# kaleo996/F5E-TTS

Measured on AMD Instinct MI355X. Metric: mel_frames_per_sec, higher is better.
Workload: dtype bf16; 1 GPU; C2: F5TTS_v1_Base random-init, batch 1 per GPU, N_ref=188 N=469 frames, euler NFE=32, CFG=2.0 (cond+uncond batched), sway=-1.0, hipGraph ODE loop, HIP log-mel front-end + Vocos decode on GPU; parallelism=replica x1 (utterance sharding, no collective on the data path)

## Files before the change

f5e-tts_amd/csrc/attention.hip:

```cpp
#include <cstdlib>
#include "attention_step.h"

namespace {

struct AttnArgs {
  const bf16* q; const bf16* k; const bf16* v;
  bf16* o; int ldo;
  const int* kv_len;
  int S, H, rows_per_seq, n_pad;
  int n_main;
  F5ePrefetch pf;
};

template <int NSPLIT>
__global__ __launch_bounds__(NSPLIT * 64, 2) void attn_fwd_kernel(AttnArgs a) {
  __shared__ __attribute__((aligned(16))) float red[(NSPLIT > 1 ? NSPLIT - 1 : 1) * 64 * 34];

  const int lane = threadIdx.x & 63;
  const int wave = __builtin_amdgcn_readfirstlane(threadIdx.x >> 6);
  const int ql = lane & 31, hh = lane >> 5;
  if ((int)blockIdx.x >= a.n_main) {
    f5e_prefetch_run<NSPLIT * 64>(a.pf, (int)blockIdx.x - a.n_main, threadIdx.x, red);
    return;
  }

  const int qtiles = (a.rows_per_seq + 31) / 32;
  int bid = blockIdx.x;
  {
    const int nblk = a.n_main;
    const int q8 = nblk >> 3, r8 = nblk & 7;
    const int xcd = bid & 7, idx = bid >> 3;
    bid = (xcd < r8 ? xcd * (q8 + 1) : r8 * (q8 + 1) + (xcd - r8) * q8) + idx;
  }
  const int qt = bid % qtiles;
  bid /= qtiles;
  const int head = bid % a.H;
  const int seq = bid / a.H;
  const size_t sh = (size_t)seq * a.H + head;
  const int kv_len = a.kv_len ? min(a.kv_len[seq], a.rows_per_seq) : a.rows_per_seq;
  const int ntiles = (kv_len + 63) / 64;

  const bf16* Qg = a.q + sh * a.n_pad * 64;
  const bf16* Kg = a.k + sh * a.n_pad * 64;
  const bf16* Vg = a.v + sh * a.n_pad * 64;

  bf16x8 qf[4];
#pragma unroll
  for (int ks = 0; ks < 4; ++ks) qf[ks] = *(const bf16x8*)(Qg + ((size_t)(qt * 4 + ks) * 32 + ql) * 16 + hh * 8);

  bf16x8 kf[2][4], vf[2][2][2];
  auto load_tile = [&](int t64) {
#pragma unroll
    for (int t = 0; t < 2; ++t) {
      const size_t tile = (size_t)t64 * 2 + t;
#pragma unroll
      for (int ks = 0; ks < 4; ++ks) kf[t][ks] = *(const bf16x8*)(Kg + ((tile * 4 + ks) * 32 + ql) * 16 + hh * 8);
#pragma unroll
      for (int s = 0; s < 2; ++s)
#pragma unroll
        for (int dt = 0; dt < 2; ++dt)
          vf[t][s][dt] = *(const bf16x8*)(Vg + ((((tile * 2 + s) * 2 + dt) * 32 + ql) * 2 + hh) * 8);
    }
  };

  f32x16 oacc[2], minit;
  float m_run, l_val;
  bf16x8 ck[2][4], cv[2][2][2];
  int t64;
  auto advance = [&]() -> int {
#pragma unroll
    for (int t = 0; t < 2; ++t) {
#pragma unroll
      for (int ks = 0; ks < 4; ++ks) ck[t][ks] = kf[t][ks];
#pragma unroll
      for (int s = 0; s < 2; ++s)
#pragma unroll
        for (int dt = 0; dt < 2; ++dt) cv[t][s][dt] = vf[t][s][dt];
    }
    const int cur = t64;
    t64 += NSPLIT;
    if (t64 < ntiles) load_tile(t64);
    return cur;
  };
  auto pass_begin = [&]() {
#pragma unroll
    for (int r = 0; r < 16; ++r) { oacc[0][r] = 0.f; oacc[1][r] = 0.f; minit[r] = 0.f; }
    m_run = -INFINITY;
    l_val = 0.f;
    t64 = wave;
    if (t64 < ntiles) load_tile(t64);
  };
  auto checked_tile = [&](bool first) {
    const int cur = advance();
    f32x16 st[2];
    auto qk = [&](f32x16 (&d)[2], const f32x16& c) {
#pragma unroll
      for (int t = 0; t < 2; ++t) {
        d[t] = __builtin_amdgcn_mfma_f32_32x32x16_bf16(ck[t][0], qf[0], c, 0, 0, 0);
#pragma unroll
        for (int ks = 1; ks < 4; ++ks) d[t] = __builtin_amdgcn_mfma_f32_32x32x16_bf16(ck[t][ks], qf[ks], d[t], 0, 0, 0);
      }
    };
    softmax_step(qk, first, cur * 64 + 64 > kv_len, cur * 64 + 4 * hh, kv_len, st, minit, m_run, l_val, oacc);
#pragma unroll
    for (int t = 0; t < 2; ++t)
#pragma unroll
      for (int s = 0; s < 2; ++s) {
        bf16x8 pf;
#pragma unroll
        for (int j = 0; j < 8; ++j) pf[j] = (bf16)st[t][8 * s + j];
#pragma unroll
        for (int dt = 0; dt < 2; ++dt)
          oacc[dt] = __builtin_amdgcn_mfma_f32_32x32x16_bf16(cv[t][s][dt], pf, oacc[dt], 0, 0, 0);
      }
  };

  pass_begin();
  if (t64 < ntiles) checked_tile(true);
  const int nfull = (ntiles * 64 > kv_len) ? ntiles - 1 : ntiles;
  while (t64 < nfull) {
    advance();
    auto kfrag = [&](int t, int ks) { return ck[t][ks]; };
    auto vfrag = [&](int t, int s, int dt) { return cv[t][s][dt]; };
    fast_step(kfrag, vfrag, qf, minit, l_val, oacc);
  }
  if (t64 < ntiles) checked_tile(false);
  if (__builtin_amdgcn_ballot_w64(!accum_finite(l_val, oacc)) != 0) {
    pass_begin();
    bool first = true;
    while (t64 < ntiles) { checked_tile(first); first = false; }
  }

  float l_run = add_xor32(l_val);
  if (NSPLIT > 1) {
    if (wave > 0) {
      f32x4* dq = (f32x4*)(red + (wave - 1) * 64 * 34);
#pragma unroll
      for (int g = 0; g < 4; ++g) {
        dq[g * 64 + lane] = f32x4{oacc[0][4 * g], oacc[0][4 * g + 1], oacc[0][4 * g + 2], oacc[0][4 * g + 3]};
        dq[(4 + g) * 64 + lane] = f32x4{oacc[1][4 * g], oacc[1][4 * g + 1], oacc[1][4 * g + 2], oacc[1][4 * g + 3]};
      }
      *(f32x2*)(red + (wave - 1) * 64 * 34 + 64 * 32 + lane * 2) = f32x2{m_run, l_run};
    }
    __syncthreads();
    if (wave > 0) return;
#pragma unroll
    for (int w = 1; w < NSPLIT; ++w) {
      const f32x4* sq = (const f32x4*)(red + (w - 1) * 64 * 34);
      const f32x2 ml = *(const f32x2*)(red + (w - 1) * 64 * 34 + 64 * 32 + lane * 2);
      const float m_new = fmaxf(m_run, ml[0]);
      const float fa = fast_exp2(m_run - m_new), fb = fast_exp2(ml[0] - m_new);
#pragma unroll
      for (int g = 0; g < 4; ++g) {
        const f32x4 s0 = sq[g * 64 + lane], s1 = sq[(4 + g) * 64 + lane];
#pragma unroll
        for (int r = 0; r < 4; ++r) {
          oacc[0][4 * g + r] = oacc[0][4 * g + r] * fa + s0[r] * fb;
          oacc[1][4 * g + r] = oacc[1][4 * g + r] * fa + s1[r] * fb;
        }
      }
      l_run = l_run * fa + ml[1] * fb;
      m_run = m_new;
    }
  }

  {
    const float inv = l_run > 0.f ? 1.0f / l_run : 0.f;
    char* stg = (char*)red;
    if (NSPLIT > 1) asm volatile("s_waitcnt lgkmcnt(0)" ::: "memory");
#pragma unroll
    for (int dt = 0; dt < 2; ++dt)
#pragma unroll
      for (int g = 0; g < 4; ++g)
        *(bf16x4*)(stg + ql * 144 + 64 * dt + 16 * g + 8 * hh) =
            f2bf4(oacc[dt][4 * g] * inv, oacc[dt][4 * g + 1] * inv, oacc[dt][4 * g + 2] * inv, oacc[dt][4 * g + 3] * inv);
    asm volatile("s_waitcnt lgkmcnt(0)" ::: "memory");
#pragma unroll
    for (int it = 0; it < 4; ++it) {
      const int r = it * 8 + (lane >> 3), c = lane & 7;
      const int q_row = qt * 32 + r;
      const uint4 v = *(const uint4*)(stg + r * 144 + c * 16);
      if (q_row < a.rows_per_seq)
        *(uint4*)(a.o + ((size_t)seq * a.rows_per_seq + q_row) * a.ldo + head * 64 + c * 8) = v;
    }
  }
}


template <int NST, int OCC>
__global__ __launch_bounds__(256, OCC) void attn_fwd_lds_kernel(AttnArgs a) {
  constexpr int TILE_BYTES = 16384;
  extern __shared__ __attribute__((aligned(16))) char smem[];

  const int tid = threadIdx.x;
  const int lane = tid & 63;
  const int wave = __builtin_amdgcn_readfirstlane(tid >> 6);
  const int ql = lane & 31, hh = lane >> 5;

  const int qblocks = (a.rows_per_seq + 127) / 128;
  int bid = blockIdx.x;
  {
    const int nblk = gridDim.x;
    const int q8 = nblk >> 3, r8 = nblk & 7;
    const int xcd = bid & 7, idx = bid >> 3;
    bid = (xcd < r8 ? xcd * (q8 + 1) : r8 * (q8 + 1) + (xcd - r8) * q8) + idx;
  }
  const int qb = bid % qblocks;
  bid /= qblocks;
  const int head = bid % a.H;
  const int seq = bid / a.H;
  const size_t sh = (size_t)seq * a.H + head;
  const int kv_len = a.kv_len ? min(a.kv_len[seq], a.rows_per_seq) : a.rows_per_seq;
  const int ntiles = (kv_len + 63) / 64;

  const bf16* Qg = a.q + sh * a.n_pad * 64;
  const char* Kg = (const char*)(a.k + sh * a.n_pad * 64);
  const char* Vg = (const char*)(a.v + sh * a.n_pad * 64);

  const int qt = min(qb * 4 + wave, a.n_pad / 32 - 1);
  bf16x8 qf[4];
#pragma unroll
  for (int ks = 0; ks < 4; ++ks) qf[ks] = *(const bf16x8*)(Qg + ((size_t)(qt * 4 + ks) * 32 + ql) * 16 + hh * 8);

  const int src16 = ((lane & 31) * 2 + (lane >> 5)) * 16;
  auto stage = [&](int buf, int t64) {
    char* dst = smem + buf * TILE_BYTES;
#pragma unroll
    for (int j = 0; j < 2; ++j) {
      const int off = (wave * 64 + 256 * j) * 16;
      __builtin_amdgcn_global_load_lds((const __attribute__((address_space(1))) void*)(Kg + (size_t)t64 * 8192 + off + src16),
                                       (__attribute__((address_space(3))) void*)(dst + off), 16, 0, 0);
      __builtin_amdgcn_global_load_lds((const __attribute__((address_space(1))) void*)(Vg + (size_t)t64 * 8192 + off + src16),
                                       (__attribute__((address_space(3))) void*)(dst + 8192 + off), 16, 0, 0);
    }
  };

  f32x16 oacc[2], minit;
  float m_run, l_val;

  int buf = 0, nbuf = NST - 1;
  auto tile_wait = [&](int t64) -> const char* {
    const int young = min(NST - 2, ntiles - 1 - t64);
    if (young >= 2) asm volatile("s_waitcnt vmcnt(8) lgkmcnt(0)" ::: "memory");
    else if (young == 1) asm volatile("s_waitcnt vmcnt(4) lgkmcnt(0)" ::: "memory");
    else asm volatile("s_waitcnt vmcnt(0) lgkmcnt(0)" ::: "memory");
    __builtin_amdgcn_s_barrier();
    return smem + buf * TILE_BYTES;
  };
  auto tile_stage = [&](int t64) {
    if (t64 + NST - 1 < ntiles) stage(nbuf, t64 + NST - 1);
    buf = (buf == NST - 1) ? 0 : buf + 1;
    nbuf = (nbuf == NST - 1) ? 0 : nbuf + 1;
  };
  auto tile_begin = [&](int t64) -> const char* {
    const char* Ks = tile_wait(t64);
    tile_stage(t64);
    return Ks;
  };
  auto pass_begin = [&]() {
#pragma unroll
    for (int r = 0; r < 16; ++r) { oacc[0][r] = 0.f; oacc[1][r] = 0.f; minit[r] = 0.f; }
    m_run = -INFINITY;
    l_val = 0.f;
    buf = 0;
    nbuf = NST - 1;
#pragma unroll
    for (int t = 0; t < NST - 1; ++t)
      if (t < ntiles) stage(t, t);
  };
  auto checked_tile = [&](int t64) {
    const char* Ks = tile_begin(t64);
    const char* Vs = Ks + 8192;
    f32x16 st[2];
    auto qk = [&](f32x16 (&d)[2], const f32x16& c) {
#pragma unroll
      for (int ks = 0; ks < 4; ++ks)
#pragma unroll
        for (int t = 0; t < 2; ++t) {
          const bf16x8 kf = *(const bf16x8*)(Ks + (t * 4 + ks) * 1024 + lane * 16);
          d[t] = __builtin_amdgcn_mfma_f32_32x32x16_bf16(kf, qf[ks], ks == 0 ? c : d[t], 0, 0, 0);
        }
    };
    softmax_step(qk, t64 == 0, t64 * 64 + 64 > kv_len, t64 * 64 + 4 * hh, kv_len, st, minit, m_run, l_val, oacc);
#pragma unroll
    for (int t = 0; t < 2; ++t)
#pragma unroll
      for (int s = 0; s < 2; ++s) {
        bf16x8 pf;
#pragma unroll
        for (int j = 0; j < 8; ++j) pf[j] = (bf16)st[t][8 * s + j];
#pragma unroll
        for (int dt = 0; dt < 2; ++dt) {
          const bf16x8 vf = *(const bf16x8*)(Vs + (((t * 2 + s) * 2 + dt) * 1024) + lane * 16);
          oacc[dt] = __builtin_amdgcn_mfma_f32_32x32x16_bf16(vf, pf, oacc[dt], 0, 0, 0);
        }
      }
  };

  pass_begin();
  if (ntiles > 0) checked_tile(0);
  const int nfull = (ntiles > 0 && ntiles * 64 > kv_len) ? ntiles - 1 : ntiles;
  for (int t64 = 1; t64 < nfull; ++t64) {
    const char* Ks = tile_wait(t64);
    const char* Vs = Ks + 8192;
    bf16x8 kf0[4];
#pragma unroll
    for (int ks = 0; ks < 4; ++ks) kf0[ks] = *(const bf16x8*)(Ks + ks * 1024 + lane * 16);
    tile_stage(t64);
    auto kfrag = [&](int t, int ks) { return t == 0 ? kf0[ks] : *(const bf16x8*)(Ks + (t * 4 + ks) * 1024 + lane * 16); };
    auto vfrag = [&](int t, int s, int dt) { return *(const bf16x8*)(Vs + (((t * 2 + s) * 2 + dt) * 1024) + lane * 16); };
    fast_step(kfrag, vfrag, qf, minit, l_val, oacc);
  }
  if (nfull < ntiles && ntiles > 1) checked_tile(ntiles - 1);
  if (__syncthreads_or(!accum_finite(l_val, oacc))) {
    pass_begin();
    for (int t64 = 0; t64 < ntiles; ++t64) checked_tile(t64);
  }

  const float l_run = add_xor32(l_val);
  const int q_row = (qb * 4 + wave) * 32 + ql;
  if (q_row < a.rows_per_seq) {
    const float inv = l_run > 0.f ? 1.0f / l_run : 0.f;
    bf16* op = a.o + ((size_t)seq * a.rows_per_seq + q_row) * a.ldo + head * 64 + 4 * hh;
#pragma unroll
    for (int dt = 0; dt < 2; ++dt)
#pragma unroll
      for (int g = 0; g < 4; ++g) {
        *(bf16x4*)(op + dt * 32 + 8 * g) = f2bf4(oacc[dt][4 * g] * inv, oacc[dt][4 * g + 1] * inv,
                                                   oacc[dt][4 * g + 2] * inv, oacc[dt][4 * g + 3] * inv);
      }
  }
}

}

int f5e_flash_attn_pf(hipStream_t st, const void* q, const void* k, const void* v, void* o, int ldo, const int* kv_len,
                      int S, int H, int rows_per_seq, int n_pad, int splits, const F5ePrefetch* pf) {
  F5E_REQUIRE(q && k && v && o, "flash_attn: null pointer");
  F5E_REQUIRE(S > 0 && H > 0 && rows_per_seq > 0, "flash_attn: empty problem");
  F5E_REQUIRE(n_pad % 64 == 0 && n_pad >= rows_per_seq, "flash_attn: n_pad=%d must be a multiple of 64 and >= %d",
              n_pad, rows_per_seq);
  F5E_REQUIRE(ldo % 8 == 0 && ldo >= H * 64 && ((uintptr_t)o & 15) == 0, "flash_attn: bad ldo=%d / output alignment", ldo);
  AttnArgs a{};
  a.q = (const bf16*)q; a.k = (const bf16*)k; a.v = (const bf16*)v; a.o = (bf16*)o; a.ldo = ldo;
  a.kv_len = kv_len; a.S = S; a.H = H; a.rows_per_seq = rows_per_seq; a.n_pad = n_pad;
  const int grid = ((rows_per_seq + 31) / 32) * H * S;
  a.n_main = grid;
  if (splits == -1 || (splits == 0 && grid >= 8192)) {
    const int g128 = ((rows_per_seq + 127) / 128) * H * S;
#ifdef F5E_TOOLS
    static const int variant = getenv("F5E_ATTN_VARIANT") ? atoi(getenv("F5E_ATTN_VARIANT")) : 0;
    if (variant == 33) {
      static F5eDeviceOnce once33;
      hipLaunchKernelGGL((attn_fwd_lds_kernel<3, 3>), dim3(g128), dim3(256), 3 * 16384, st, a);
    } else if (variant == 23) {
      hipLaunchKernelGGL((attn_fwd_lds_kernel<2, 3>), dim3(g128), dim3(256), 2 * 16384, st, a);
    } else if (variant == 42) {
      hipLaunchKernelGGL((attn_fwd_lds_kernel<4, 2>), dim3(g128), dim3(256), 4 * 16384, st, a);
    } else
#endif
    hipLaunchKernelGGL((attn_fwd_lds_kernel<2, 4>), dim3(g128), dim3(256), 2 * 16384, st, a);
    F5E_LAUNCH_CHECK("flash_attn_lds");
    return F5E_OK;
  }
  if (splits <= 0) {
    const int ktiles = (rows_per_seq + 63) / 64;
    splits = grid > 2 * f5e_cu_count() ? 1 : 4;
    while (splits > 1 && splits > ktiles) splits >>= 1;
  }
  switch (splits) {
    case 1: {
      const int npf = f5e_prefetch_wgs(pf);
      if (npf) a.pf = *pf;
      hipLaunchKernelGGL(attn_fwd_kernel<1>, dim3(grid + npf), dim3(64), 0, st, a);
      break;
    }
    case 2: {
      const int npf = f5e_prefetch_wgs(pf);
      if (npf) a.pf = *pf;
      hipLaunchKernelGGL(attn_fwd_kernel<2>, dim3(grid + npf), dim3(128), 0, st, a);
      break;
    }
    case 4: {
      const int npf = f5e_prefetch_wgs(pf);
      if (npf) a.pf = *pf;
      hipLaunchKernelGGL(attn_fwd_kernel<4>, dim3(grid + npf), dim3(256), 0, st, a);
      break;
    }
    default: F5E_REQUIRE(false, "flash_attn: splits must be 0 (auto), -1 (LDS-shared), 1, 2 or 4");
  }
  F5E_LAUNCH_CHECK("flash_attn");
  return F5E_OK;
}

extern "C" int f5e_flash_attn(hipStream_t st, const void* q, const void* k, const void* v, void* o, int ldo,
                              const int* kv_len, int S, int H, int rows_per_seq, int n_pad, int splits) {
  return f5e_flash_attn_pf(st, q, k, v, o, ldo, kv_len, S, H, rows_per_seq, n_pad, splits, nullptr);
}
```

include/f5e_abi.h:

```cpp
#ifndef F5E_ABI_H_
#define F5E_ABI_H_

#ifdef __cplusplus
extern "C" {
#endif

#define F5E_ABI_VERSION 2

#if defined(__GNUC__)
#define F5E_API __attribute__((visibility("default")))
#else
#define F5E_API
#endif

enum { F5E_OK = 0, F5E_ERR_BAD_SHAPE = -1, F5E_ERR_UNSUPPORTED = -2, F5E_ERR_HIP = -3 };

enum { F5E_ACT_NONE = 0, F5E_ACT_SILU = 1, F5E_ACT_GELU_ERF = 2, F5E_ACT_GELU_TANH = 3, F5E_ACT_RELU = 4, F5E_ACT_MISH = 5 };

#ifdef F5E_STREAM_T
typedef F5E_STREAM_T f5e_stream;
#else
typedef void* f5e_stream;
#endif

F5E_API int f5e_abi_version(void);
F5E_API const char* f5e_last_error(void);
F5E_API int f5e_check_device(void);


F5E_API int f5e_gemm_bf16_bias(f5e_stream st, const void* A, int lda, const void* W, int ldw, const float* bias, void* out,
                       int ldo, int M, int N, int K, int act, int out_f32, int tile_hint);

F5E_API int f5e_gemm_bf16_gate_residual(f5e_stream st, const void* A, int lda, const void* W, int ldw, const float* bias,
                                float* resid, int ldr, const float* gate, int gate_stride, int gate_rows,
                                const int* eval_ptr, int eval_stride, int rows_per_seq, const int* seq_len, int M,
                                int N, int K, int tile_hint);

F5E_API int f5e_gemm_bf16_qkv_rope(f5e_stream st, const void* A, int lda, const void* W, int ldw, const float* bias, void* q,
                           void* k, void* vt, int n_pad, int heads, int rope_heads, const float* cos_sin,
                           const float* q_norm_w, const float* k_norm_w, int rows_per_seq, int M, int K,
                           int tile_hint);

typedef struct f5e_ln_fuse {
  const float* stats; int parts;
  const float* c; const float* d; int cd_stride; int cd_rows; int cd_eval_stride;
  const int* eval_ptr; int rows_per_seq; float eps;
  void* xs_out; int ld_xs; const float* next_scale;
  float* stats_out;
  float* row_mean;
} f5e_ln_fuse;

F5E_API int f5e_gemm_bf16_bias_ln(f5e_stream st, const void* A, int lda, const void* W, int ldw, const float* bias, void* out,
                          int ldo, int M, int N, int K, int act, int out_f32, int tile_hint, const f5e_ln_fuse* ln);
F5E_API int f5e_gemm_bf16_gate_residual_ln(f5e_stream st, const void* A, int lda, const void* W, int ldw, const float* bias,
                                   float* resid, int ldr, const float* gate, int gate_stride, int gate_rows,
                                   const int* eval_ptr, int eval_stride, int rows_per_seq, const int* seq_len, int M,
                                   int N, int K, int tile_hint, const f5e_ln_fuse* ln);
F5E_API int f5e_gemm_bf16_qkv_rope_ln(f5e_stream st, const void* A, int lda, const void* W, int ldw, const float* bias,
                              void* q, void* k, void* vt, int n_pad, int heads, int rope_heads, const float* cos_sin,
                              const float* q_norm_w, const float* k_norm_w, int rows_per_seq, int M, int K,
                              int tile_hint, const f5e_ln_fuse* ln);


F5E_API int f5e_flash_attn(f5e_stream st, const void* q, const void* k, const void* vt, void* o, int ldo, const int* kv_len,
                   int S, int H, int rows_per_seq, int n_pad, int splits);

F5E_API int f5e_joint_attn(f5e_stream st, const void* qx, const void* kx, const void* vx, const void* qc, const void* kc,
                   const void* vc, void* o_x, int ldo_x, void* o_c, int ldo_c, const int* kv_len, int S, int H, int N,
                   int n_pad_x, int Nt, int n_pad_c, int splits);


F5E_API int f5e_layernorm(f5e_stream st, const float* x, int ldx, void* y, int ldy, int y_bf16, const float* gamma,
                  const float* beta, const float* scale, const float* shift, int mod_stride, int mod_rows,
                  int rows_per_seq, const int* eval_ptr, int eval_stride, int rows, int D, float eps);

F5E_API int f5e_adaln_pre(f5e_stream st, const float* x, int ldx, void* xs, int ld_xs, const float* scale, int mod_stride,
                  int mod_rows, int rows_per_seq, const int* eval_ptr, int eval_stride, float* stats, int parts,
                  float* row_mean, int rows, int D);

F5E_API int f5e_l2norm(f5e_stream st, const float* x, int ldx, void* y, int ldy, int y_bf16, const float* g, int rows, int D);

F5E_API int f5e_grn(f5e_stream st, const float* x, float* y, float* gx_ws, const float* gamma, const float* beta, int B, int T,
            int C);


F5E_API int f5e_gemm_f32(f5e_stream st, const float* A, int lda, int a_rows, int a_act, const float* W, int ldw,
                 const float* bias, int act, const float* ch_scale, const float* addend, int ld_add, int add_rows,
                 const float* row_scale, float* out, int ldo, void* out_bf16, int ldo_bf16, int M, int N, int K);


F5E_API int f5e_convpos(f5e_stream st, const void* x, int ldx, const void* w_packed, const float* bias, int mode,
                void* out_bf16, int ldo, float* out_f32, int ldo32, const float* resid, int ldr, int S, int N, int D,
                int groups);

F5E_API int f5e_dwconv7(f5e_stream st, const float* x, const float* w_t, const float* bias, float* y, int B, int T, int C);

F5E_API int f5e_im2col(f5e_stream st, const float* x, float* col, int B, int T, int Cin, int ksize, int pad);


F5E_API int f5e_sinus_embed(f5e_stream st, const float* t, const float* freqs, float* out, int E, int dim, float scale);
F5E_API int f5e_rope_table(f5e_stream st, const float* inv_freq, float* out, int N, int half);
F5E_API int f5e_text_gather(f5e_stream st, const int* ids, const float* table, const float* pos, const float* keep, float* out,
                    int B, int N, int TD, int max_pos, int table_rows);
F5E_API int f5e_ode_update(f5e_stream st, const float* pred, long long branch_stride, int mode, float w0, float w1,
                   const float* base, float* dst, float* traj, const float* coef, int* eval_ptr, unsigned* done_ctr,
                   long long n);
F5E_API int f5e_ode_update_traj(f5e_stream st, const float* pred, long long branch_stride, int mode, float w0, float w1,
                        const float* base, float* dst, float* traj, long long traj_stride, int traj_div,
                        const float* coef, int* eval_ptr, unsigned* done_ctr, long long n);
F5E_API int f5e_advance_eval(f5e_stream st, int* eval_ptr);
F5E_API int f5e_stitch(f5e_stream st, const float* cond, const float* y, const unsigned char* mask, float* out, long long rows,
               int C);
F5E_API int f5e_cast_bf16(f5e_stream st, const float* x, void* y, long long n);
F5E_API int f5e_cast_f32(f5e_stream st, const void* x, float* y, long long n);
F5E_API int f5e_axpby(f5e_stream st, const float* x, const float* y, float* out, float a, float b, float c, long long n);
F5E_API int f5e_vq_eval(f5e_stream st, const float* logits, int ld, const float* vars, int combine_groups, float* out,
                int* targets, float* stats, int rows, int groups, int num_vars, int var_dim);

F5E_API int f5e_mas_workspace_bytes(int B, int Ty, int Tx, unsigned long long* bytes_out_host);
F5E_API int f5e_mas_path(f5e_stream st, const float* logp, long long batch_stride, int ld, const int* t_y, const int* t_x,
                 int* token_of_frame, int* durations, void* workspace, unsigned long long workspace_bytes, int B, int Ty,
                 int Tx);

F5E_API int f5e_resample(f5e_stream st, const float* x, long long ld_x, const float* bank, int orig, int new_, int width,
                 float* y, long long ld_y, int B, int n, int n_out);

F5E_API int f5e_ctc_align_workspace_bytes(int B, int T, int L, unsigned long long* bytes_out_host);
F5E_API int f5e_ctc_align(f5e_stream st, const float* scores, long long batch_stride, int ld, const int* labels, int ld_labels,
                  const int* t_len, const int* l_len, int blank, int* align, int* tok_start, int* tok_end, float* score,
                  void* workspace, unsigned long long workspace_bytes, int B, int T, int L, int V);

F5E_API int f5e_ctc_greedy(f5e_stream st, const float* scores, long long batch_stride, int ld, const int* t_len, int blank,
                   int pad_id, int* hyp, int* hyp_len, float* frame_logp, int B, int T, int V);

F5E_API int f5e_ctc_beam_workspace_bytes(int B, int T, int beam, unsigned long long* bytes_out_host);
F5E_API int f5e_ctc_beam(f5e_stream st, const float* scores, long long batch_stride, int ld, const int* t_len, int blank,
                 int beam, int* hyp, int ld_hyp, int* hyp_len, float* score, void* workspace,
                 unsigned long long workspace_bytes, int B, int T, int V);

F5E_API int f5e_ctc_beam_state_bytes(int B, int T_cap, int chunk_cap, int beam, unsigned long long* bytes_out_host);
F5E_API int f5e_ctc_beam_state_init(f5e_stream st, void* state, unsigned long long state_bytes, int B, int T_cap,
                            int chunk_cap, int beam);
F5E_API int f5e_ctc_beam_chunk(f5e_stream st, const float* scores, long long batch_stride, int ld, const int* n_frames,
                       int T_chunk, int V, int blank, int beam, void* state, unsigned long long state_bytes, int* hyp,
                       int ld_hyp, int* hyp_len, float* score, int B, int T_cap, int chunk_cap);

F5E_API int f5e_token_logp(f5e_stream st, const float* logits, long long ld, const int* target, float* out, long long rows,
                   int V);
F5E_API int f5e_log_softmax_rows(f5e_stream st, const float* x, long long ldx, float* out, long long ldo, long long rows,
                         int V);


F5E_API int f5e_stft_logmel(f5e_stream st, const float* wav, int nw, int ldw, const float* window, const float* twiddle,
                    const float* fb, float* out, int B, int n_fft, int hop, int n_mels);
F5E_API int f5e_stft_logmel_banded(f5e_stream st, const float* wav, int nw, int ldw, const float* window, const float* twiddle,
                           const float* fb_compact, const int* fb_band, int nnz, float* out, int B, int n_fft, int hop,
                           int n_mels);
F5E_API int f5e_stft_logmel_banded_ex(f5e_stream st, const float* wav, int nw, int ldw, const float* window,
                              const float* twiddle, const float* fb_compact, const int* fb_band, int nnz, float* out, int B,
                              int n_fft, int hop, int n_mels, int pad_left, int T, float mag_eps);
F5E_API int f5e_istft_head(f5e_stream st, const float* z, int ldz, const float* window, const float* twiddle, float* frames_ws,
                   float* out, int B, int T, int n_fft, int hop);


F5E_API int f5e_bigvgan_act(f5e_stream st, const float* x, void* y, int out_f32, const float* alpha, const float* inv_beta,
                    const float* f_up, const float* f_dn, int B, int L, int C);
F5E_API int f5e_bigvgan_conv(f5e_stream st, const void* x, const void* w_packed, const float* bias, const float* resid,
                     float* out, float* sum, float sum_scale, int sum_init, int B, int L, int Cin, int Cin_pad, int N,
                     int ksz, int dil, int pad);
F5E_API int f5e_bigvgan_post(f5e_stream st, const float* a, const float* w, const float* bias, float* out, int B, int L, int C,
                     int ksz, int use_tanh);


F5E_API int f5e_kaldi_fbank(f5e_stream st, const float* wav, int nw, int ldw, const float* window, const float* twiddle,
                    const float* fb, float* out, int B, int win, int shift, int n_mels, float in_scale, float preemph,
                    float eps);
F5E_API int f5e_glu(f5e_stream st, const float* x, int ldx, float* y, int ldy, long long rows, int C);
F5E_API int f5e_dwconv(f5e_stream st, const float* x, const float* w_t, const float* bias, const float* keep, float* y, int B,
               int T, int C, int K);
F5E_API int f5e_softmax_rows(f5e_stream st, const float* x, int ldx, float* y, int ldy, const int* kv_len, long long rows,
                     int rows_per_seq, int L, float scale);
F5E_API int f5e_dwconv_stream(f5e_stream st, const float* x, const float* w_t, const float* bias, const float* fill, float* y,
                      int B, int T, int C, int K, int causal, int chunk);
F5E_API int f5e_relpos_attn(f5e_stream st, const float* qu, int ldq, const float* k, int ldk, const float* pos, int ldp,
                    const float* v, int ldv, float* out, int ldo, const int* kv_len, int B, int T, int H, int dk,
                    int q_begin, int chunk, int left_chunks, float scale);
F5E_API int f5e_mha_f32(f5e_stream st, const float* q, int ldq, const float* k, int ldk, const float* v, int ldv, float* out,
                int ldo, const int* kv_len, int B, int Tq, int Tk, int H, int dk, int causal, float scale);

F5E_API int f5e_attn_decode_f32(f5e_stream st, const float* qkv, int ld_qkv, float* kc, float* vc, long long row_stride,
                        int pos_stride, const int* anc, int ld_anc, float* out, int ldo, int R, int Umax, int H, int dk, int p,
                        float scale);
F5E_API int f5e_beam_step(f5e_stream st, const float* logits, long long ld_logits, float* score, const int* hyp_in,
                  const int* anc_in, int* hyp_out, int* anc_out, int ld, int* last, int* alive, int* done_at, int B, int V,
                  int beam, int p, int eos);


typedef struct f5e_dit_block_weights {
  const void* w_qkv;  const float* b_qkv;
  const void* w_out;  const float* b_out;
  const void* w_ff1;  const float* b_ff1;
  const void* w_ff2;  const float* b_ff2;
  const float* q_norm_w; const float* k_norm_w;
} f5e_dit_block_weights;

typedef struct f5e_dit_plan {
  int S, B, N, n_pad, D, H, rope_heads, FF, L, mel;
  int mod_rows;
  const float* y;
  const float* w_x; int ldw_x;
  const float* in_const;
  const void* convpos_w1; const float* convpos_b1;
  const void* convpos_w2; const float* convpos_b2;
  int convpos_groups;
  const float* rope_cs;
  const int* seq_len;
  const float* mod;
  const int* eval_ptr;
  const f5e_dit_block_weights* blocks;
  const void* w_proj; const float* b_proj;
  const float* w_skip;
  float* skip_res; float* skip_tmp;
  float* h0; void* h0_bf16; void* c1;
  float* x;
  void* hn;
  void* q; void* k; void* vt;
  void* ao;
  void* ff;
  float* pred;
  void* timer;
  int timer_op;
  int fuse_ln;
  float* ln_stats;
  float* ln_rowmean;
  const float* cd;
  int cd_stride;
  int mall_prefetch;
} f5e_dit_plan;

enum { F5E_WS_H0 = 0, F5E_WS_H0_BF16, F5E_WS_C1, F5E_WS_X, F5E_WS_HN, F5E_WS_Q, F5E_WS_K, F5E_WS_VT, F5E_WS_AO, F5E_WS_FF,
       F5E_WS_PRED, F5E_WS_LN_STATS, F5E_WS_SKIP_RES, F5E_WS_SKIP_TMP, F5E_WS_LN_ROWMEAN, F5E_WS_COUNT };
typedef struct f5e_dit_workspace {
  int n_pad;
  unsigned long long bytes[F5E_WS_COUNT];
  unsigned long long offset[F5E_WS_COUNT];
  unsigned long long total;
} f5e_dit_workspace;
F5E_API int f5e_workspace_bytes(const f5e_dit_plan* shape, f5e_dit_workspace* out_host);

enum { F5E_OP_NONE = 0, F5E_OP_INPROJ = 1, F5E_OP_CONVPOS = 2, F5E_OP_LN = 3, F5E_OP_QKV = 4, F5E_OP_ATTN = 5,
       F5E_OP_OUT = 6, F5E_OP_FF1 = 7, F5E_OP_FF2 = 8, F5E_OP_FINAL = 9 };

F5E_API int f5e_timer_create(int capacity, void** timer_out);
F5E_API int f5e_timer_destroy(void* timer);
F5E_API int f5e_timer_reset(void* timer);
F5E_API int f5e_timer_read(void* timer, float* ms_out_host, int max_out, int* count_out_host);
F5E_API int f5e_timer_read_ops(void* timer, int* ops_out_host, int max_out, int* count_out_host);

#ifdef F5E_TOOLS
F5E_API void f5e_debug_convpos_trace(void* buf);
#endif

F5E_API int f5e_dit_forward(f5e_stream st, const f5e_dit_plan* plan);

typedef struct f5e_loop_plan {
  const f5e_dit_plan* eval_a;
  const f5e_dit_plan* eval_b;
  int steps;
  int mode; float w0, w1;
  long long n;
  float* y;
  float* y_mid;
  const float* pred;
  const float* coef;
  int* eval_ptr;
  unsigned* done_ctr;
  float* traj;
} f5e_loop_plan;
F5E_API int f5e_sample_loop(f5e_stream st, const f5e_loop_plan* loop);

F5E_API int f5e_graph_begin(f5e_stream st);
F5E_API int f5e_graph_end(f5e_stream st, void** graph_exec_out);
F5E_API int f5e_graph_launch(void* graph_exec, f5e_stream st);
F5E_API int f5e_graph_destroy(void* graph_exec);

#ifdef __cplusplus
}
#endif
#endif
```

Before: 13010 mel-frames/s.

## Add two-tile-per-wave attention kernel with upfront K/V loads and parallel merge

Adds a specialized split-4 attention kernel for short sequences (at most 8 KV tiles). Each wave issues all of its K/V tile loads at kernel entry, before reading kv_len, so global memory latency overlaps. The cross-wave softmax merge is spread across all four waves instead of serialized on wave 0. The change also adds s_memtime trace instrumentation, compiled only under the tools build. The trade-off is higher register use from holding two tiles of K/V fragments, and loads of clamped tiles even when a wave owns no work.

After: 13220 mel-frames/s (median of 6 runs). 1.02x the previous value.

```diff
diff --git a/f5e-tts_amd/csrc/attention.hip b/f5e-tts_amd/csrc/attention.hip
--- a/f5e-tts_amd/csrc/attention.hip
+++ b/f5e-tts_amd/csrc/attention.hip
@@ -10,9 +10,44 @@
   int S, H, rows_per_seq, n_pad;
   int n_main;
   F5ePrefetch pf;
+#ifdef F5E_TOOLS
+  unsigned long long* trace;
+#endif
 };
 
-template <int NSPLIT>
+#ifdef F5E_TOOLS
+#define ATTN_STAMP(i)                                                                                    \
+  do {                                                                                                   \
+    if constexpr (TRC) {                                                                                 \
+      __builtin_amdgcn_sched_barrier(0);                                                                 \
+      asm volatile("s_memtime %0\n\ts_waitcnt lgkmcnt(0)" : "=s"(ts[i]) :: "memory");                    \
+      __builtin_amdgcn_sched_barrier(0);                                                                 \
+    }                                                                                                    \
+  } while (0)
+#define ATTN_LANDED(n, i)                                                                                \
+  do {                                                                                                   \
+    if constexpr (TRC) {                                                                                 \
+      __builtin_amdgcn_sched_barrier(0);                                                                 \
+      asm volatile("s_waitcnt vmcnt(" #n ")\n\ts_memtime %0\n\ts_waitcnt lgkmcnt(0)" : "=s"(ts[i]) :: "memory"); \
+      __builtin_amdgcn_sched_barrier(0);                                                                 \
+    }                                                                                                    \
+  } while (0)
+#define ATTN_TRACE_OUT()                                                                                 \
+  do {                                                                                                   \
+    if constexpr (TRC) {                                                                                 \
+      if (lane == 0 && a.trace) {                                                                        \
+        unsigned long long* tp = a.trace + ((size_t)blockIdx.x * (blockDim.x >> 6) + wave) * 8;          \
+        for (int i = 0; i < 8; ++i) tp[i] = ts[i];                                                       \
+      }                                                                                                  \
+    }                                                                                                    \
+  } while (0)
+#else
+#define ATTN_STAMP(i) do {} while (0)
+#define ATTN_LANDED(n, i) do {} while (0)
+#define ATTN_TRACE_OUT() do {} while (0)
+#endif
+
+template <int NSPLIT, bool TRC = false>
 __global__ __launch_bounds__(NSPLIT * 64, 2) void attn_fwd_kernel(AttnArgs a) {
   __shared__ __attribute__((aligned(16))) float red[(NSPLIT > 1 ? NSPLIT - 1 : 1) * 64 * 34];
 
@@ -23,6 +58,8 @@
     f5e_prefetch_run<NSPLIT * 64>(a.pf, (int)blockIdx.x - a.n_main, threadIdx.x, red);
     return;
   }
+  [[maybe_unused]] unsigned long long ts[8] = {};
+  ATTN_STAMP(0);
 
   const int qtiles = (a.rows_per_seq + 31) / 32;
   int bid = blockIdx.x;
@@ -91,6 +128,7 @@
     if (t64 < ntiles) load_tile(t64);
   };
   auto checked_tile = [&](bool first) {
+    if (first) { ATTN_LANDED(0, 2); } else { ATTN_LANDED(0, 3); }
     const int cur = advance();
     f32x16 st[2];
     auto qk = [&](f32x16 (&d)[2], const f32x16& c) {
@@ -119,6 +157,7 @@
   if (t64 < ntiles) checked_tile(true);
   const int nfull = (ntiles * 64 > kv_len) ? ntiles - 1 : ntiles;
   while (t64 < nfull) {
+    ATTN_LANDED(0, 3);
     advance();
     auto kfrag = [&](int t, int ks) { return ck[t][ks]; };
     auto vfrag = [&](int t, int s, int dt) { return cv[t][s][dt]; };
@@ -142,8 +181,13 @@
       }
       *(f32x2*)(red + (wave - 1) * 64 * 34 + 64 * 32 + lane * 2) = f32x2{m_run, l_run};
     }
+    ATTN_STAMP(4);
     __syncthreads();
-    if (wave > 0) return;
+    ATTN_STAMP(5);
+    if (wave > 0) {
+      ATTN_TRACE_OUT();
+      return;
+    }
 #pragma unroll
     for (int w = 1; w < NSPLIT; ++w) {
       const f32x4* sq = (const f32x4*)(red + (w - 1) * 64 * 34);
@@ -184,6 +228,181 @@
         *(uint4*)(a.o + ((size_t)seq * a.rows_per_seq + q_row) * a.ldo + head * 64 + c * 8) = v;
     }
   }
+  ATTN_STAMP(6);
+  ATTN_TRACE_OUT();
+}
+
+template <bool TRC>
+__global__ __launch_bounds__(256, 2) void attn_fwd_b1_kernel(AttnArgs a) {
+  constexpr int NSPLIT = 4, PART = 64 * 34;
+  __shared__ __attribute__((aligned(16))) float red[NSPLIT * PART + 32 * 36];
+
+  const int lane = threadIdx.x & 63;
+  const int wave = __builtin_amdgcn_readfirstlane(threadIdx.x >> 6);
+  const int ql = lane & 31, hh = lane >> 5;
+  if ((int)blockIdx.x >= a.n_main) {
+    f5e_prefetch_run<NSPLIT * 64>(a.pf, (int)blockIdx.x - a.n_main, threadIdx.x, red);
+    return;
+  }
+  __builtin_amdgcn_s_waitcnt(0x0070);
+  [[maybe_unused]] unsigned long long ts[8] = {};
+  ATTN_STAMP(0);
+
+  const int qtiles = (a.rows_per_seq + 31) / 32;
+  int bid = blockIdx.x;
+  {
+    const int nblk = a.n_main;
+    const int q8 = nblk >> 3, r8 = nblk & 7;
+    const int xcd = bid & 7, idx = bid >> 3;
+    bid = (xcd < r8 ? xcd * (q8 + 1) : r8 * (q8 + 1) + (xcd - r8) * q8) + idx;
+  }
+  const int qt = bid % qtiles;
+  bid /= qtiles;
+  const int head = bid % a.H;
+  const int seq = bid / a.H;
+  const size_t sh = (size_t)seq * a.H + head;
+
+  const bf16* Qg = a.q + sh * a.n_pad * 64;
+  const bf16* Kg = a.k + sh * a.n_pad * 64;
+  const bf16* Vg = a.v + sh * a.n_pad * 64;
+
+  bf16x8 qf[4];
+#pragma unroll
+  for (int ks = 0; ks < 4; ++ks) qf[ks] = *(const bf16x8*)(Qg + ((size_t)(qt * 4 + ks) * 32 + ql) * 16 + hh * 8);
+  bf16x8 kf[2][2][4], vf[2][2][2][2];
+  const int last64 = a.n_pad / 64 - 1;
+  auto load_k = [&](int st) {
+    const int t64 = min(wave + st * NSPLIT, last64);
+#pragma unroll
+    for (int t = 0; t < 2; ++t)
+#pragma unroll
+      for (int ks = 0; ks < 4; ++ks)
+        kf[st][t][ks] = *(const bf16x8*)(Kg + ((((size_t)t64 * 2 + t) * 4 + ks) * 32 + ql) * 16 + hh * 8);
+  };
+  auto load_v = [&](int st) {
+    const int t64 = min(wave + st * NSPLIT, last64);
+#pragma unroll
+    for (int t = 0; t < 2; ++t)
+#pragma unroll
+      for (int s = 0; s < 2; ++s)
+#pragma unroll
+        for (int dt = 0; dt < 2; ++dt)
+          vf[st][t][s][dt] = *(const bf16x8*)(Vg + ((((((size_t)t64 * 2 + t) * 2 + s) * 2 + dt) * 32 + ql) * 2 + hh) * 8);
+  };
+  load_k(0);
+  load_v(0);
+  load_k(1);
+  load_v(1);
+  const int kv_len = a.kv_len ? min(load_uniform_i32(a.kv_len + seq), a.rows_per_seq) : a.rows_per_seq;
+  const int ntiles = (kv_len + 63) / 64;
+  ATTN_LANDED(32, 1);
+  ATTN_LANDED(16, 2);
+
+  f32x16 oacc[2], minit;
+  float m_run, l_val;
+  auto pass_begin = [&]() {
+#pragma unroll
+    for (int r = 0; r < 16; ++r) { oacc[0][r] = 0.f; oacc[1][r] = 0.f; minit[r] = 0.f; }
+    m_run = -INFINITY;
+    l_val = 0.f;
+  };
+  auto checked_tile = [&](const bf16x8 (&ck)[2][4], const bf16x8 (&cv)[2][2][2], int cur, bool first) {
+    f32x16 st[2];
+    auto qk = [&](f32x16 (&d)[2], const f32x16& c) {
+#pragma unroll
+      for (int t = 0; t < 2; ++t) {
+        d[t] = __builtin_amdgcn_mfma_f32_32x32x16_bf16(ck[t][0], qf[0], c, 0, 0, 0);
+#pragma unroll
+        for (int ks = 1; ks < 4; ++ks) d[t] = __builtin_amdgcn_mfma_f32_32x32x16_bf16(ck[t][ks], qf[ks], d[t], 0, 0, 0);
+      }
+    };
+    softmax_step(qk, first, cur * 64 + 64 > kv_len, cur * 64 + 4 * hh, kv_len, st, minit, m_run, l_val, oacc);
+#pragma unroll
+    for (int t = 0; t < 2; ++t)
+#pragma unroll
+      for (int s = 0; s < 2; ++s) {
+        bf16x8 pf;
+#pragma unroll
+        for (int j = 0; j < 8; ++j) pf[j] = (bf16)st[t][8 * s + j];
+#pragma unroll
+        for (int dt = 0; dt < 2; ++dt)
+          oacc[dt] = __builtin_amdgcn_mfma_f32_32x32x16_bf16(cv[t][s][dt], pf, oacc[dt], 0, 0, 0);
+      }
+  };
+
+  const bool own0 = wave < ntiles, own1 = wave + NSPLIT < ntiles;
+  const int nfull = (ntiles * 64 > kv_len) ? ntiles - 1 : ntiles;
+  pass_begin();
+  if (own0) checked_tile(kf[0], vf[0], wave, true);
+  if (own1) {
+    ATTN_LANDED(0, 3);
+    if (wave + NSPLIT < nfull) {
+      auto kfrag = [&](int t, int ks) { return kf[1][t][ks]; };
+      auto vfrag = [&](int t, int s, int dt) { return vf[1][t][s][dt]; };
+      fast_step(kfrag, vfrag, qf, minit, l_val, oacc);
+    } else {
+      checked_tile(kf[1], vf[1], wave + NSPLIT, false);
+    }
+  }
+  if (__builtin_amdgcn_ballot_w64(!accum_finite(l_val, oacc)) != 0) {
+    pass_begin();
+    load_k(0);
+    load_v(0);
+    load_k(1);
+    load_v(1);
+    if (own0) checked_tile(kf[0], vf[0], wave, true);
+    if (own1) checked_tile(kf[1], vf[1], wave + NSPLIT, false);
+  }
+
+  {
+    const float l_w = add_xor32(l_val);
+    f32x4* dq = (f32x4*)(red + wave * PART);
+#pragma unroll
+    for (int g = 0; g < 4; ++g) {
+      dq[g * 64 + lane] = f32x4{oacc[0][4 * g], oacc[0][4 * g + 1], oacc[0][4 * g + 2], oacc[0][4 * g + 3]};
+      dq[(4 + g) * 64 + lane] = f32x4{oacc[1][4 * g], oacc[1][4 * g + 1], oacc[1][4 * g + 2], oacc[1][4 * g + 3]};
+    }
+    *(f32x2*)(red + wave * PART + 64 * 32 + lane * 2) = f32x2{m_run, l_w};
+  }
+  ATTN_STAMP(4);
+  __syncthreads();
+  ATTN_STAMP(5);
+
+  char* stg = (char*)(red + NSPLIT * PART);
+  {
+    const int g = wave;
+    f32x4 o0 = ((const f32x4*)red)[g * 64 + lane], o1 = ((const f32x4*)red)[(4 + g) * 64 + lane];
+    const f32x2 ml0 = *(const f32x2*)(red + 64 * 32 + lane * 2);
+    float m_mrg = ml0[0], l_run = ml0[1];
+#pragma unroll
+    for (int w = 1; w < NSPLIT; ++w) {
+      const f32x4* sq = (const f32x4*)(red + w * PART);
+      const f32x2 ml = *(const f32x2*)(red + w * PART + 64 * 32 + lane * 2);
+      const float m_new = fmaxf(m_mrg, ml[0]);
+      const float fa = fast_exp2(m_mrg - m_new), fb = fast_exp2(ml[0] - m_new);
+      const f32x4 s0 = sq[g * 64 + lane], s1 = sq[(4 + g) * 64 + lane];
+#pragma unroll
+      for (int r = 0; r < 4; ++r) {
+        o0[r] = o0[r] * fa + s0[r] * fb;
+        o1[r] = o1[r] * fa + s1[r] * fb;
+      }
+      l_run = l_run * fa + ml[1] * fb;
+      m_mrg = m_new;
+    }
+    const float inv = l_run > 0.f ? 1.0f / l_run : 0.f;
+    *(bf16x4*)(stg + ql * 144 + 16 * g + 8 * hh) = f2bf4(o0[0] * inv, o0[1] * inv, o0[2] * inv, o0[3] * inv);
+    *(bf16x4*)(stg + ql * 144 + 64 + 16 * g + 8 * hh) = f2bf4(o1[0] * inv, o1[1] * inv, o1[2] * inv, o1[3] * inv);
+  }
+  __syncthreads();
+  {
+    const int r = wave * 8 + (lane >> 3), c = lane & 7;
+    const int q_row = qt * 32 + r;
+    const uint4 v = *(const uint4*)(stg + r * 144 + c * 16);
+    if (q_row < a.rows_per_seq)
+      *(uint4*)(a.o + ((size_t)seq * a.rows_per_seq + q_row) * a.ldo + head * 64 + c * 8) = v;
+  }
+  ATTN_STAMP(6);
+  ATTN_TRACE_OUT();
 }
 
 
@@ -333,6 +552,11 @@
 }
 
 }
+
+#ifdef F5E_TOOLS
+static unsigned long long* g_attn_trace = nullptr;
+extern "C" void f5e_debug_attn_trace(void* buf) { g_attn_trace = (unsigned long long*)buf; }
+#endif
 
 int f5e_flash_attn_pf(hipStream_t st, const void* q, const void* k, const void* v, void* o, int ldo, const int* kv_len,
                       int S, int H, int rows_per_seq, int n_pad, int splits, const F5ePrefetch* pf) {
@@ -384,7 +608,24 @@
     case 4: {
       const int npf = f5e_prefetch_wgs(pf);
       if (npf) a.pf = *pf;
-      hipLaunchKernelGGL(attn_fwd_kernel<4>, dim3(grid + npf), dim3(256), 0, st, a);
+      const bool two_steps = (rows_per_seq + 63) / 64 <= 8;
+#ifdef F5E_TOOLS
+      static const int variant4 = getenv("F5E_ATTN_VARIANT") ? atoi(getenv("F5E_ATTN_VARIANT")) : 0;
+      a.trace = g_attn_trace;
+      if (a.trace || variant4 == 4) {
+        if (two_steps && variant4 != 4) {
+          if (a.trace) hipLaunchKernelGGL(attn_fwd_b1_kernel<true>, dim3(grid + npf), dim3(256), 0, st, a);
+          else hipLaunchKernelGGL(attn_fwd_b1_kernel<false>, dim3(grid + npf), dim3(256), 0, st, a);
+        } else if (a.trace) {
+          hipLaunchKernelGGL((attn_fwd_kernel<4, true>), dim3(grid + npf), dim3(256), 0, st, a);
+        } else {
+          hipLaunchKernelGGL(attn_fwd_kernel<4>, dim3(grid + npf), dim3(256), 0, st, a);
+        }
+        break;
+      }
+#endif
+      if (two_steps) hipLaunchKernelGGL(attn_fwd_b1_kernel<false>, dim3(grid + npf), dim3(256), 0, st, a);
+      else hipLaunchKernelGGL(attn_fwd_kernel<4>, dim3(grid + npf), dim3(256), 0, st, a);
       break;
     }
     default: F5E_REQUIRE(false, "flash_attn: splits must be 0 (auto), -1 (LDS-shared), 1, 2 or 4");
diff --git a/include/f5e_abi.h b/include/f5e_abi.h
--- a/include/f5e_abi.h
+++ b/include/f5e_abi.h
@@ -259,6 +259,7 @@
 
 #ifdef F5E_TOOLS
 F5E_API void f5e_debug_convpos_trace(void* buf);
+F5E_API void f5e_debug_attn_trace(void* buf);
 #endif
 
 F5E_API int f5e_dit_forward(f5e_stream st, const f5e_dit_plan* plan);
```
